# nagadomi/nunif

Measured on NVIDIA H100. Metric: waifu2x_input_megapixels_per_sec, higher is better.
Workload: dtype f16

## Files before the change

### nunif_b200/csrc/gemm_wgmma.cuh

```cuda
#pragma once
#include "common.cuh"
#include "ptx.cuh"
#include <cuda.h>

namespace nb200 {

enum : int { ACT_NONE = 0, ACT_LRELU01 = 1, ACT_GELU = 2, ACT_RELU = 3 };
enum : int { OUT_NHWC = 0, OUT_PIXSHUF2 = 1, OUT_SPLIT = 2 };

struct GemmParams {
    int B, Ho, Wo, TH, TW, tiles_x, tiles_y;
    int N;
    int taps, cpt;
    int8_t tap_dx[16], tap_dy[16], tap_dyi[16];
    int n_tiles;
    const float* bias;
    int act;
    int out_mode, cout;
    int has_res, res_cy, res_cx;
    int res_before_act;
    int k2;
};

struct GemmMaps {
    CUtensorMap a, b;
    CUtensorMap o[4];
    union {
        CUtensorMap r[4];
        CUtensorMap a2;
    };
};

__device__ __forceinline__ void mbar_init(uint64_t* bar, uint32_t count) {
    asm volatile("mbarrier.init.shared::cta.b64 [%0], %1;" ::"r"(smem_u32(bar)), "r"(count));
}
__device__ __forceinline__ void mbar_expect_tx(uint64_t* bar, uint32_t bytes) {
    asm volatile("mbarrier.arrive.expect_tx.shared::cta.b64 _, [%0], %1;" ::"r"(smem_u32(bar)), "r"(bytes) : "memory");
}
__device__ __forceinline__ void mbar_arrive(uint64_t* bar) {
    asm volatile("mbarrier.arrive.shared::cta.b64 _, [%0];" ::"r"(smem_u32(bar)) : "memory");
}
__device__ __forceinline__ void mbar_wait(uint64_t* bar, uint32_t parity) {
    const uint32_t addr = smem_u32(bar);
    uint32_t done = 0;
#pragma unroll 1
    for (uint32_t it = 0; it < (1u << 18) && !done; ++it)
        asm volatile(
            "{\n\t.reg .pred p;\n\t"
            "mbarrier.try_wait.parity.shared::cta.b64 p, [%1], %2, %3;\n\t"
            "selp.u32 %0, 1, 0, p;\n\t}"
            : "=r"(done) : "r"(addr), "r"(parity), "r"(20000u) : "memory");
    if (!done) __trap();
}
__device__ __forceinline__ void fence_barrier_init() {
    asm volatile("fence.mbarrier_init.release.cluster;" ::: "memory");
    asm volatile("fence.proxy.async.shared::cta;" ::: "memory");
}
__device__ __forceinline__ void tma_load_5d(const CUtensorMap* map, uint64_t* bar, void* dst, int c0, int c1, int c2, int c3, int c4) {
    asm volatile(
        "cp.async.bulk.tensor.5d.shared::cluster.global.tile.mbarrier::complete_tx::bytes [%0], [%1, {%3, %4, %5, %6, %7}], [%2];"
        ::"r"(smem_u32(dst)), "l"(map), "r"(smem_u32(bar)), "r"(c0), "r"(c1), "r"(c2), "r"(c3), "r"(c4) : "memory");
}
__device__ __forceinline__ void tma_load_2d(const CUtensorMap* map, uint64_t* bar, void* dst, int c0, int c1) {
    asm volatile(
        "cp.async.bulk.tensor.2d.shared::cluster.global.tile.mbarrier::complete_tx::bytes [%0], [%1, {%3, %4}], [%2];"
        ::"r"(smem_u32(dst)), "l"(map), "r"(smem_u32(bar)), "r"(c0), "r"(c1) : "memory");
}
__device__ __forceinline__ void tma_load_4d(const CUtensorMap* map, uint64_t* bar, void* dst, int c0, int c1, int c2, int c3) {
    asm volatile(
        "cp.async.bulk.tensor.4d.shared::cluster.global.tile.mbarrier::complete_tx::bytes [%0], [%1, {%3, %4, %5, %6}], [%2];"
        ::"r"(smem_u32(dst)), "l"(map), "r"(smem_u32(bar)), "r"(c0), "r"(c1), "r"(c2), "r"(c3) : "memory");
}
__device__ __forceinline__ void tma_store_4d(const CUtensorMap* map, const void* src, int c0, int c1, int c2, int c3) {
    asm volatile("cp.async.bulk.tensor.4d.global.shared::cta.tile.bulk_group [%0, {%2, %3, %4, %5}], [%1];"
                 ::"l"(map), "r"(smem_u32(src)), "r"(c0), "r"(c1), "r"(c2), "r"(c3) : "memory");
}
__device__ __forceinline__ void tma_store_2d(const CUtensorMap* map, const void* src, int c0, int c1) {
    asm volatile("cp.async.bulk.tensor.2d.global.shared::cta.tile.bulk_group [%0, {%2, %3}], [%1];"
                 ::"l"(map), "r"(smem_u32(src)), "r"(c0), "r"(c1) : "memory");
}
__device__ __forceinline__ void tma_store_commit() { asm volatile("cp.async.bulk.commit_group;" ::: "memory"); }
__device__ __forceinline__ void tma_store_wait_read() { asm volatile("cp.async.bulk.wait_group.read 0;" ::: "memory"); }
__device__ __forceinline__ void fence_async_smem() { asm volatile("fence.proxy.async.shared::cta;" ::: "memory"); }
__device__ __forceinline__ void consumer_bar_sync() { asm volatile("bar.sync 1, 256;" ::: "memory"); }
__device__ __forceinline__ void tma_prefetch_desc(const CUtensorMap* map) {
    asm volatile("prefetch.tensormap [%0];" ::"l"(map) : "memory");
}
__device__ __forceinline__ bool elect_one() {
    uint32_t pred;
    asm volatile(
        "{\n\t.reg .pred p;\n\t"
        "elect.sync _|p, 0xffffffff;\n\t"
        "selp.u32 %0, 1, 0, p;\n\t}"
        : "=r"(pred));
    return pred != 0;
}
__device__ __forceinline__ void wgmma_fence() { asm volatile("wgmma.fence.sync.aligned;" ::: "memory"); }
__device__ __forceinline__ void wgmma_commit() { asm volatile("wgmma.commit_group.sync.aligned;" ::: "memory"); }
template <int N>
__device__ __forceinline__ void wgmma_wait() { asm volatile("wgmma.wait_group.sync.aligned %0;" ::"n"(N) : "memory"); }
template <int K>
__device__ __forceinline__ void wgmma_fence_operands(float (&d)[K]) {
#pragma unroll
    for (int j = 0; j < K; ++j) asm volatile("" : "+f"(d[j])::"memory");
}

template <int SWIZZLE_BYTES>
__device__ __forceinline__ uint64_t make_kmajor_desc(uint32_t saddr) {
    constexpr uint64_t layout = SWIZZLE_BYTES == 128 ? 1 : (SWIZZLE_BYTES == 64 ? 2 : 3);
    constexpr uint64_t sbo = (8 * SWIZZLE_BYTES) >> 4;
    return (uint64_t)((saddr & 0x3FFFF) >> 4) | (1ull << 16) | (sbo << 32) | (layout << 62);
}

template <int N>
__device__ void wgmma_f16(float (&d)[N / 2], uint64_t a, uint64_t b, uint32_t acc);
template <> __device__ __forceinline__ void wgmma_f16<16>(float (&d)[8], uint64_t a, uint64_t b, uint32_t acc) {
    asm volatile("{\n\t.reg .pred p;\n\tsetp.ne.b32 p, %10, 0;\n\t"
                 "wgmma.mma_async.sync.aligned.m64n16k16.f32.f16.f16 {%0, %1, %2, %3, %4, %5, %6, %7}, %8, %9, p, 1, 1, 0, 0;\n\t}"
                 : "+f"(d[0]), "+f"(d[1]), "+f"(d[2]), "+f"(d[3]), "+f"(d[4]), "+f"(d[5]), "+f"(d[6]), "+f"(d[7])
                 : "l"(a), "l"(b), "r"(acc));
}
template <> __device__ __forceinline__ void wgmma_f16<32>(float (&d)[16], uint64_t a, uint64_t b, uint32_t acc) {
    asm volatile("{\n\t.reg .pred p;\n\tsetp.ne.b32 p, %18, 0;\n\t"
                 "wgmma.mma_async.sync.aligned.m64n32k16.f32.f16.f16 {%0, %1, %2, %3, %4, %5, %6, %7, %8, %9, %10, %11, %12, %13, %14, %15}, %16, %17, p, 1, 1, 0, 0;\n\t}"
                 : "+f"(d[0]), "+f"(d[1]), "+f"(d[2]), "+f"(d[3]), "+f"(d[4]), "+f"(d[5]), "+f"(d[6]), "+f"(d[7]), "+f"(d[8]), "+f"(d[9]), "+f"(d[10]), "+f"(d[11]), "+f"(d[12]), "+f"(d[13]), "+f"(d[14]), "+f"(d[15])
                 : "l"(a), "l"(b), "r"(acc));
}
template <> __device__ __forceinline__ void wgmma_f16<48>(float (&d)[24], uint64_t a, uint64_t b, uint32_t acc) {
    asm volatile("{\n\t.reg .pred p;\n\tsetp.ne.b32 p, %26, 0;\n\t"
                 "wgmma.mma_async.sync.aligned.m64n48k16.f32.f16.f16 {%0, %1, %2, %3, %4, %5, %6, %7, %8, %9, %10, %11, %12, %13, %14, %15, %16, %17, %18, %19, %20, %21, %22, %23}, %24, %25, p, 1, 1, 0, 0;\n\t}"
                 : "+f"(d[0]), "+f"(d[1]), "+f"(d[2]), "+f"(d[3]), "+f"(d[4]), "+f"(d[5]), "+f"(d[6]), "+f"(d[7]), "+f"(d[8]), "+f"(d[9]), "+f"(d[10]), "+f"(d[11]), "+f"(d[12]), "+f"(d[13]), "+f"(d[14]), "+f"(d[15]), "+f"(d[16]), "+f"(d[17]), "+f"(d[18]), "+f"(d[19]), "+f"(d[20]), "+f"(d[21]), "+f"(d[22]), "+f"(d[23])
                 : "l"(a), "l"(b), "r"(acc));
}
template <> __device__ __forceinline__ void wgmma_f16<64>(float (&d)[32], uint64_t a, uint64_t b, uint32_t acc) {
    asm volatile("{\n\t.reg .pred p;\n\tsetp.ne.b32 p, %34, 0;\n\t"
                 "wgmma.mma_async.sync.aligned.m64n64k16.f32.f16.f16 {%0, %1, %2, %3, %4, %5, %6, %7, %8, %9, %10, %11, %12, %13, %14, %15, %16, %17, %18, %19, %20, %21, %22, %23, %24, %25, %26, %27, %28, %29, %30, %31}, %32, %33, p, 1, 1, 0, 0;\n\t}"
                 : "+f"(d[0]), "+f"(d[1]), "+f"(d[2]), "+f"(d[3]), "+f"(d[4]), "+f"(d[5]), "+f"(d[6]), "+f"(d[7]), "+f"(d[8]), "+f"(d[9]), "+f"(d[10]), "+f"(d[11]), "+f"(d[12]), "+f"(d[13]), "+f"(d[14]), "+f"(d[15]), "+f"(d[16]), "+f"(d[17]), "+f"(d[18]), "+f"(d[19]), "+f"(d[20]), "+f"(d[21]), "+f"(d[22]), "+f"(d[23]), "+f"(d[24]), "+f"(d[25]), "+f"(d[26]), "+f"(d[27]), "+f"(d[28]), "+f"(d[29]), "+f"(d[30]), "+f"(d[31])
                 : "l"(a), "l"(b), "r"(acc));
}
template <> __device__ __forceinline__ void wgmma_f16<96>(float (&d)[48], uint64_t a, uint64_t b, uint32_t acc) {
    asm volatile("{\n\t.reg .pred p;\n\tsetp.ne.b32 p, %50, 0;\n\t"
                 "wgmma.mma_async.sync.aligned.m64n96k16.f32.f16.f16 {%0, %1, %2, %3, %4, %5, %6, %7, %8, %9, %10, %11, %12, %13, %14, %15, %16, %17, %18, %19, %20, %21, %22, %23, %24, %25, %26, %27, %28, %29, %30, %31, %32, %33, %34, %35, %36, %37, %38, %39, %40, %41, %42, %43, %44, %45, %46, %47}, %48, %49, p, 1, 1, 0, 0;\n\t}"
                 : "+f"(d[0]), "+f"(d[1]), "+f"(d[2]), "+f"(d[3]), "+f"(d[4]), "+f"(d[5]), "+f"(d[6]), "+f"(d[7]), "+f"(d[8]), "+f"(d[9]), "+f"(d[10]), "+f"(d[11]), "+f"(d[12]), "+f"(d[13]), "+f"(d[14]), "+f"(d[15]), "+f"(d[16]), "+f"(d[17]), "+f"(d[18]), "+f"(d[19]), "+f"(d[20]), "+f"(d[21]), "+f"(d[22]), "+f"(d[23]), "+f"(d[24]), "+f"(d[25]), "+f"(d[26]), "+f"(d[27]), "+f"(d[28]), "+f"(d[29]), "+f"(d[30]), "+f"(d[31]), "+f"(d[32]), "+f"(d[33]), "+f"(d[34]), "+f"(d[35]), "+f"(d[36]), "+f"(d[37]), "+f"(d[38]), "+f"(d[39]), "+f"(d[40]), "+f"(d[41]), "+f"(d[42]), "+f"(d[43]), "+f"(d[44]), "+f"(d[45]), "+f"(d[46]), "+f"(d[47])
                 : "l"(a), "l"(b), "r"(acc));
}
template <> __device__ __forceinline__ void wgmma_f16<128>(float (&d)[64], uint64_t a, uint64_t b, uint32_t acc) {
    asm volatile("{\n\t.reg .pred p;\n\tsetp.ne.b32 p, %66, 0;\n\t"
                 "wgmma.mma_async.sync.aligned.m64n128k16.f32.f16.f16 {%0, %1, %2, %3, %4, %5, %6, %7, %8, %9, %10, %11, %12, %13, %14, %15, %16, %17, %18, %19, %20, %21, %22, %23, %24, %25, %26, %27, %28, %29, %30, %31, %32, %33, %34, %35, %36, %37, %38, %39, %40, %41, %42, %43, %44, %45, %46, %47, %48, %49, %50, %51, %52, %53, %54, %55, %56, %57, %58, %59, %60, %61, %62, %63}, %64, %65, p, 1, 1, 0, 0;\n\t}"
                 : "+f"(d[0]), "+f"(d[1]), "+f"(d[2]), "+f"(d[3]), "+f"(d[4]), "+f"(d[5]), "+f"(d[6]), "+f"(d[7]), "+f"(d[8]), "+f"(d[9]), "+f"(d[10]), "+f"(d[11]), "+f"(d[12]), "+f"(d[13]), "+f"(d[14]), "+f"(d[15]), "+f"(d[16]), "+f"(d[17]), "+f"(d[18]), "+f"(d[19]), "+f"(d[20]), "+f"(d[21]), "+f"(d[22]), "+f"(d[23]), "+f"(d[24]), "+f"(d[25]), "+f"(d[26]), "+f"(d[27]), "+f"(d[28]), "+f"(d[29]), "+f"(d[30]), "+f"(d[31]), "+f"(d[32]), "+f"(d[33]), "+f"(d[34]), "+f"(d[35]), "+f"(d[36]), "+f"(d[37]), "+f"(d[38]), "+f"(d[39]), "+f"(d[40]), "+f"(d[41]), "+f"(d[42]), "+f"(d[43]), "+f"(d[44]), "+f"(d[45]), "+f"(d[46]), "+f"(d[47]), "+f"(d[48]), "+f"(d[49]), "+f"(d[50]), "+f"(d[51]), "+f"(d[52]), "+f"(d[53]), "+f"(d[54]), "+f"(d[55]), "+f"(d[56]), "+f"(d[57]), "+f"(d[58]), "+f"(d[59]), "+f"(d[60]), "+f"(d[61]), "+f"(d[62]), "+f"(d[63])
                 : "l"(a), "l"(b), "r"(acc));
}

__device__ __forceinline__ void wgmma_f16_rs96(float (&d)[48], const uint32_t (&a)[4], uint64_t b, uint32_t acc) {
    asm volatile("{\n\t.reg .pred p;\n\tsetp.ne.b32 p, %53, 0;\n\t"
                 "wgmma.mma_async.sync.aligned.m64n96k16.f32.f16.f16 {%0, %1, %2, %3, %4, %5, %6, %7, %8, %9, %10, %11, %12, %13, %14, %15, %16, %17, %18, %19, %20, %21, %22, %23, %24, %25, %26, %27, %28, %29, %30, %31, %32, %33, %34, %35, %36, %37, %38, %39, %40, %41, %42, %43, %44, %45, %46, %47}, {%48, %49, %50, %51}, %52, p, 1, 1, 0;\n\t}"
                 : "+f"(d[0]), "+f"(d[1]), "+f"(d[2]), "+f"(d[3]), "+f"(d[4]), "+f"(d[5]), "+f"(d[6]), "+f"(d[7]), "+f"(d[8]), "+f"(d[9]), "+f"(d[10]), "+f"(d[11]), "+f"(d[12]), "+f"(d[13]), "+f"(d[14]), "+f"(d[15]), "+f"(d[16]), "+f"(d[17]), "+f"(d[18]), "+f"(d[19]), "+f"(d[20]), "+f"(d[21]), "+f"(d[22]), "+f"(d[23]), "+f"(d[24]), "+f"(d[25]), "+f"(d[26]), "+f"(d[27]), "+f"(d[28]), "+f"(d[29]), "+f"(d[30]), "+f"(d[31]), "+f"(d[32]), "+f"(d[33]), "+f"(d[34]), "+f"(d[35]), "+f"(d[36]), "+f"(d[37]), "+f"(d[38]), "+f"(d[39]), "+f"(d[40]), "+f"(d[41]), "+f"(d[42]), "+f"(d[43]), "+f"(d[44]), "+f"(d[45]), "+f"(d[46]), "+f"(d[47])
                 : "r"(a[0]), "r"(a[1]), "r"(a[2]), "r"(a[3]), "l"(b), "r"(acc));
}

__device__ __forceinline__ float gelu_erf(float x) {
    const float a = fabsf(x);
    float q = fmaf(a, 4.88118734e-04f, -7.19881030e-03f);
    q = fmaf(q, a, 5.21468017e-02f);
    q = fmaf(q, a, 4.59595724e-01f);
    q = fmaf(q, a, 1.15100057e+00f);
    const float e = ex2(fmaf(-q, a, -1.0f));
    return fmaxf(x, 0.f) - a * e;
}

template <int K>
__device__ __forceinline__ void apply_act(float (&v)[K], int act) {
    switch (act) {
        case ACT_LRELU01:
#pragma unroll
            for (int j = 0; j < K; ++j) v[j] = v[j] > 0.f ? v[j] : 0.1f * v[j];
            break;
        case ACT_GELU:
#pragma unroll
            for (int j = 0; j < K; ++j) v[j] = gelu_erf(v[j]);
            break;
        case ACT_RELU:
#pragma unroll
            for (int j = 0; j < K; ++j) v[j] = fmaxf(v[j], 0.f);
            break;
        default: break;
    }
}

constexpr int GEMM_CONSUMER_THREADS = 256;
constexpr int GEMM_THREADS = GEMM_CONSUMER_THREADS + 32;

template <int BLOCK_N, int BK>
struct GemmCfg {
    static_assert(BLOCK_N % 16 == 0 && BLOCK_N <= 128, "BLOCK_N: 16..128 (the fp32 accumulators live in registers)");
    static constexpr int SWIZZLE = BK * 2;
    static constexpr int A_BYTES = 128 * BK * 2;
    static constexpr int B_BYTES = BLOCK_N * BK * 2;
    static constexpr int STAGE_BYTES = A_BYTES + ((B_BYTES + 1023) / 1024) * 1024;
    static constexpr int STAGES = (98304 / STAGE_BYTES) < 2 ? 2 : ((98304 / STAGE_BYTES) > 6 ? 6 : (98304 / STAGE_BYTES));
    static constexpr int CW = (BLOCK_N % 64 == 0) ? 64 : ((BLOCK_N % 32 == 0) ? 32 : 16);
    static constexpr int NCH = BLOCK_N / CW;
    static constexpr int CH_BYTES = 128 * CW * 2;
    static_assert(NCH * CH_BYTES <= STAGES * STAGE_BYTES, "epilogue staging must fit in the (drained) pipeline stages");
    static constexpr int SMEM_BYTES = STAGES * STAGE_BYTES + 1024  + 256 ;
};

template <int CW>
__device__ __forceinline__ uint32_t stage_off(int r, int j) {
    if (CW == 64) return (uint32_t)(r * 128 + ((j ^ (r & 7)) << 4));
    if (CW == 32) return (uint32_t)(r * 64 + ((j ^ ((r >> 1) & 3)) << 4));
    return (uint32_t)(r * 32 + ((j ^ ((r >> 2) & 1)) << 4));
}

template <int ROWS>
__device__ __forceinline__ uint32_t sw64_off(int r, int col) {
    return (uint32_t)((col >> 5) * (ROWS * 64)) + stage_off<32>(r, (col & 31) >> 3) + (uint32_t)((col & 7) * 2);
}

template <int BLOCK_N, int BK, bool A2 = false>
__global__ void __launch_bounds__(GEMM_THREADS, 2) gemm_conv_kernel(const __grid_constant__ GemmMaps maps,
                                                                    const __grid_constant__ GemmParams p) {
    using Cfg = GemmCfg<BLOCK_N, BK>;
    constexpr int STAGES = Cfg::STAGES;
    constexpr int CW = Cfg::CW;
    extern __shared__ uint8_t smem_dyn[];
    uint8_t* smem = reinterpret_cast<uint8_t*>((reinterpret_cast<uintptr_t>(smem_dyn) + 1023) & ~(uintptr_t)1023);
    uint64_t* full_bar = reinterpret_cast<uint64_t*>(smem + STAGES * Cfg::STAGE_BYTES);
    uint64_t* empty_bar = full_bar + STAGES;
    uint64_t* res_bar = empty_bar + STAGES;

    const int warp = threadIdx.x >> 5;
    const int n_tile = blockIdx.x % p.n_tiles;
    const int tile = blockIdx.x / p.n_tiles;
    const int tx_i = tile % p.tiles_x;
    const int ty_i = (tile / p.tiles_x) % p.tiles_y;
    const int b = tile / (p.tiles_x * p.tiles_y);
    const int x0 = tx_i * p.TW, y0 = ty_i * p.TH;
    const int n0 = n_tile * BLOCK_N;
    const int k_iters = p.taps * p.cpt + (A2 ? p.k2 : 0);

    if (threadIdx.x == GEMM_CONSUMER_THREADS) {
        tma_prefetch_desc(&maps.a);
        tma_prefetch_desc(&maps.b);
        tma_prefetch_desc(&maps.o[0]);
        for (int s = 0; s < STAGES; ++s) {
            mbar_init(&full_bar[s], 1);
            mbar_init(&empty_bar[s], 2);
        }
        mbar_init(res_bar, 1);
        fence_barrier_init();
    }
    __syncthreads();

    if (warp == GEMM_CONSUMER_THREADS / 32) {
        if (elect_one()) {
            asm volatile("griddepcontrol.wait;" ::: "memory");
            for (int it = 0; it < k_iters; ++it) {
                const int s = it % STAGES;
                const uint32_t ph = (it / STAGES) & 1;
                mbar_wait(&empty_bar[s], ph ^ 1);
                const int tap = it / p.cpt, ch = it - tap * p.cpt;
                uint8_t* sa = smem + s * Cfg::STAGE_BYTES;
                uint8_t* sb = sa + Cfg::A_BYTES;
                mbar_expect_tx(&full_bar[s], Cfg::A_BYTES + Cfg::B_BYTES);
                if (A2 && tap >= p.taps) {
                    const int q = n0 / p.cout;
                    tma_load_5d(&maps.a2, &full_bar[s], sa, (it - p.taps * p.cpt) * BK, q & 1, x0, q >> 1, b * p.Ho + y0);
                } else {
                    tma_load_5d(&maps.a, &full_bar[s], sa, ch * BK, x0 + p.tap_dx[tap], p.tap_dyi[tap], y0 + p.tap_dy[tap], b);
                }
                tma_load_2d(&maps.b, &full_bar[s], sb, it * BK, n0);
            }
        }
        return;
    }

    const int wg = threadIdx.x >> 7;
    const int t = threadIdx.x & 127;
    float acc[BLOCK_N / 2];
#pragma unroll
    for (int j = 0; j < BLOCK_N / 2; ++j) acc[j] = 0.f;
    for (int it = 0; it < k_iters; ++it) {
        const int s = it % STAGES;
        mbar_wait(&full_bar[s], (it / STAGES) & 1);
        const uint32_t sa = smem_u32(smem + s * Cfg::STAGE_BYTES) + wg * 64 * Cfg::SWIZZLE;
        const uint32_t sb = smem_u32(smem + s * Cfg::STAGE_BYTES) + Cfg::A_BYTES;
        wgmma_fence();
#pragma unroll
        for (int k = 0; k < BK / 16; ++k)
            wgmma_f16<BLOCK_N>(acc, make_kmajor_desc<Cfg::SWIZZLE>(sa + k * 32), make_kmajor_desc<Cfg::SWIZZLE>(sb + k * 32), 1u);
        wgmma_commit();
        wgmma_wait<1>();
        if (it > 0 && t == 0) mbar_arrive(&empty_bar[(it - 1) % STAGES]);
    }
    wgmma_wait<0>();
    wgmma_fence_operands(acc);
    if (threadIdx.x == 0) NB_PDL_TRIGGER();
    consumer_bar_sync();
    uint8_t* stg = smem;
    const bool leader = threadIdx.x == 0;
    if (p.has_res) {
        if (leader) {
            mbar_expect_tx(res_bar, Cfg::NCH * Cfg::CH_BYTES);
#pragma unroll 1
            for (int c = 0; c < Cfg::NCH; ++c) {
                const int n = n0 + c * CW;
                const int g = p.out_mode != OUT_NHWC ? n / p.cout : 0;
                const int co = p.out_mode != OUT_NHWC ? n - g * p.cout : n;
                tma_load_4d(&maps.r[g], res_bar, stg + c * Cfg::CH_BYTES, co, x0 + p.res_cx, y0 + p.res_cy, b);
            }
        }
        mbar_wait(res_bar, 0);
    }
    const int act = p.act;
    const bool has_res = p.has_res != 0, res_first = p.res_before_act != 0;
    const int row0 = wg * 64 + (t >> 5) * 16 + ((t & 31) >> 2);
    const int cq = 2 * (t & 3);
#pragma unroll
    for (int j = 0; j < BLOCK_N / 8; ++j) {
        const int col = 8 * j + cq;
        const int c = (8 * j) / CW;
        float2 bq = make_float2(0.f, 0.f);
        if (p.bias) bq = __ldg(reinterpret_cast<const float2*>(p.bias + n0 + col));
        float v[4] = {acc[4 * j] + bq.x, acc[4 * j + 1] + bq.y, acc[4 * j + 2] + bq.x, acc[4 * j + 3] + bq.y};
        __half2* s0 = reinterpret_cast<__half2*>(stg + c * Cfg::CH_BYTES + stage_off<CW>(row0, (8 * j % CW) / 8) + 2 * cq);
        __half2* s1 = reinterpret_cast<__half2*>(stg + c * Cfg::CH_BYTES + stage_off<CW>(row0 + 8, (8 * j % CW) / 8) + 2 * cq);
        if (has_res) {
            const float2 r0 = __half22float2(*s0), r1 = __half22float2(*s1);
            const float rv[4] = {r0.x, r0.y, r1.x, r1.y};
            if (res_first) {
#pragma unroll
                for (int q = 0; q < 4; ++q) v[q] += rv[q];
                apply_act(v, act);
            } else {
                apply_act(v, act);
#pragma unroll
                for (int q = 0; q < 4; ++q) v[q] += rv[q];
            }
        } else {
            apply_act(v, act);
        }
        *s0 = __floats2half2_rn(v[0], v[1]);
        *s1 = __floats2half2_rn(v[2], v[3]);
    }
    fence_async_smem();
    consumer_bar_sync();
    if (leader) {
#pragma unroll 1
        for (int c = 0; c < Cfg::NCH; ++c) {
            const int n = n0 + c * CW;
            const int g = p.out_mode != OUT_NHWC ? n / p.cout : 0;
            const int co = p.out_mode != OUT_NHWC ? n - g * p.cout : n;
            tma_store_4d(&maps.o[g], stg + c * Cfg::CH_BYTES, co, x0, y0, b);
        }
        tma_store_commit();
        tma_store_wait_read();
    }
}

}
```

### nunif_b200/csrc/swin_block.cu

```cuda
#include "gemm_wgmma.cuh"
#include "swin_kernels.h"
#include "tmap.h"
#include <algorithm>

namespace nb200 {

extern int g_tune[16];

constexpr int FM_ROWS = 128, FM_STAGES = 5, FM_THREADS = GEMM_CONSUMER_THREADS + 128;
constexpr int FM_PRODUCER_REGS = 40, FM_CONSUMER_REGS = 232;

template <int C>
struct FmCfg {
    static constexpr int KB = C / 32;
    static constexpr int NBUF = C == 96 ? 3 : 2;
    static constexpr int TILE = FM_ROWS * C * 2;
    static constexpr int STAGE = 128 * C;
    static constexpr int SMEM = NBUF * TILE + FM_STAGES * STAGE + (2 * FM_STAGES + NBUF * (KB + 2) + 1) * 8 + 1024;
    static_assert(SMEM <= 232448, "shared memory per CTA exceeds the opt-in limit");
};

struct FmMaps {
    CUtensorMap x, att, wp, w1, w2, y, wy;
};

template <int K>
__device__ __forceinline__ float (&half96(float (&acc)[K], int h))[48] { return *reinterpret_cast<float(*)[48]>(&acc[48 * h]); }

__device__ __forceinline__ void wgmma_wait_n(int n) {
    if (n == 0) wgmma_wait<0>();
    else wgmma_wait<1>();
}

template <int C, bool PROJ, int CS>
__global__ void __launch_bounds__(FM_THREADS, 1) swin_mlp_fused_kernel(const __grid_constant__ FmMaps maps, const float* __restrict__ bp,
                                                                     const float* __restrict__ b1, const float* __restrict__ b2,
                                                                     const float* __restrict__ by, int ntiles) {
    using Cfg = FmCfg<C>;
    static_assert(CS % 16 == 0 && 2 * C * CS <= Cfg::STAGE && CS * 256 <= Cfg::TILE, "Wy must fit a ring stage, y a tile");
    constexpr int KB = Cfg::KB, NP = (KB + 1) / 2, NH = 2 * C / 64, NHALF = C / 96, NBUF = Cfg::NBUF;
    constexpr int SPT = (PROJ ? NP : 0) + 2 * NH + (CS ? 1 : 0);
    static_assert(SPT > FM_STAGES, "the barrier protocol needs more stages per tile than the ring holds");
    constexpr int XAHEAD = PROJ ? NBUF - 1 : NBUF;
    extern __shared__ uint8_t smem_dyn[];
    uint8_t* smem = smem_dyn + ((1024u - (smem_u32(smem_dyn) & 1023u)) & 1023u);
    uint8_t* ring = smem + NBUF * Cfg::TILE;
    uint64_t* full = reinterpret_cast<uint64_t*>(ring + FM_STAGES * Cfg::STAGE);
    uint64_t* empty = full + FM_STAGES;
    uint64_t* abar = empty + FM_STAGES;
    uint64_t* xbar = abar + NBUF * KB;
    uint64_t* outw = xbar + NBUF;
    uint64_t* xfree = outw + NBUF;
    auto buf = [&](int b) { return smem + b * Cfg::TILE; };
    const int tid = threadIdx.x, warp = tid >> 5;
    const int nt = (ntiles - (int)blockIdx.x + (int)gridDim.x - 1) / (int)gridDim.x;
    if (tid == GEMM_CONSUMER_THREADS) {
        tma_prefetch_desc(&maps.x);
        tma_prefetch_desc(&maps.w1);
        tma_prefetch_desc(&maps.w2);
        if (CS) {
            tma_prefetch_desc(&maps.wy);
            tma_prefetch_desc(&maps.y);
        }
        if (PROJ) {
            tma_prefetch_desc(&maps.att);
            tma_prefetch_desc(&maps.wp);
        }
        for (int s = 0; s < FM_STAGES; ++s) {
            mbar_init(&full[s], 1);
            mbar_init(&empty[s], 2);
        }
        for (int b = 0; b < NBUF; ++b) {
            for (int kb = 0; kb < KB; ++kb) mbar_init(&abar[b * KB + kb], 1);
            mbar_init(&xbar[b], 1);
            mbar_init(&outw[b], 2);
        }
        mbar_init(xfree, 2);
        fence_barrier_init();
    }
    __syncthreads();

    if (warp >= GEMM_CONSUMER_THREADS / 32) {
        asm volatile("setmaxnreg.dec.sync.aligned.u32 %0;" ::"n"(FM_PRODUCER_REGS));
        if (warp == GEMM_CONSUMER_THREADS / 32 && elect_one()) {
            int it = 0;
            auto push = [&](const CUtensorMap* m, int k0, int n0, int rows, int nbox) {
                const int s = it % FM_STAGES;
                mbar_wait(&empty[s], ((it / FM_STAGES) & 1) ^ 1);
                mbar_expect_tx(&full[s], nbox * rows * 64);
                for (int b = 0; b < nbox; ++b) tma_load_2d(m, &full[s], ring + s * Cfg::STAGE + b * rows * 64, k0 + 32 * b, n0);
                ++it;
            };
            for (int j = 0; j < nt; ++j) {
                if (PROJ)
                    for (int p = 0; p < NP; ++p) push(&maps.wp, 64 * p, 0, C, min(2, KB - 2 * p));
                push(&maps.w1, 0, 0, 64, KB);
                for (int hc = 0; hc < NH; ++hc) {
                    if (hc + 1 < NH) push(&maps.w1, 0, (hc + 1) * 64, 64, KB);
                    push(&maps.w2, hc * 64, 0, C, 2);
                }
                if (CS) push(&maps.wy, 0, 0, CS, KB);
            }
        } else if (warp == GEMM_CONSUMER_THREADS / 32 + 1 && elect_one()) {
            auto row = [&](int j) { return ((int)blockIdx.x + j * (int)gridDim.x) * FM_ROWS; };
            auto load_att = [&](int j) {
                const int b = j % NBUF;
                for (int kb = 0; kb < KB; ++kb) {
                    mbar_expect_tx(&abar[b * KB + kb], FM_ROWS * 64);
                    tma_load_2d(&maps.att, &abar[b * KB + kb], buf(b) + kb * (FM_ROWS * 64), kb * 32, row(j));
                }
            };
            auto load_x = [&](int j) {
                uint8_t* dst = buf((j + PROJ) % NBUF);
                mbar_expect_tx(&xbar[j % NBUF], Cfg::TILE);
                for (int kb = 0; kb < KB; ++kb) tma_load_2d(&maps.x, &xbar[j % NBUF], dst + kb * (FM_ROWS * 64), kb * 32, row(j));
            };
            asm volatile("griddepcontrol.wait;" ::: "memory");
            if (PROJ) load_att(0);
            for (int j = 0; j < XAHEAD && j < nt; ++j) load_x(j);
            for (int j = 0; j < nt; ++j) {
                if (PROJ) {
                    mbar_wait(xfree, j & 1);
                    if (j + 1 < nt) load_att(j + 1);
                }
                const int b = j % NBUF;
                mbar_wait(&outw[b], (j / NBUF) & 1);
                if constexpr (CS > 0)
                    for (int c = 0; c < CS / 16; ++c) tma_store_2d(&maps.y, buf(b) + c * (FM_ROWS * 32), 16 * c, row(j));
                else
                    for (int kb = 0; kb < KB; ++kb) tma_store_2d(&maps.x, buf(b) + kb * (FM_ROWS * 64), kb * 32, row(j));
                tma_store_commit();
                tma_store_wait_read();
                if (j + XAHEAD < nt) load_x(j + XAHEAD);
            }
        }
        return;
    }

    asm volatile("setmaxnreg.inc.sync.aligned.u32 %0;" ::"n"(FM_CONSUMER_REGS));
    const int wg = tid >> 7, t = tid & 127;
    const int row0 = wg * 64 + (t >> 5) * 16 + ((t & 31) >> 2);
    const int cq = 2 * (t & 3);
#pragma unroll 1
    for (int it0 = 0; (int)blockIdx.x + it0 / SPT * (int)gridDim.x < ntiles; it0 += SPT) {
        const int j = it0 / SPT;
        int it = it0;
        const int b = j % NBUF;
        const uint32_t par = (j / NBUF) & 1;
        uint8_t* sx1 = buf(b);
        const uint8_t* sxin = buf((j + PROJ) % NBUF);
        const uint32_t x1_base = smem_u32(sx1) + wg * 64 * 64;
        int pending = 0;
        auto take = [&]() -> uint32_t {
            const int s = it % FM_STAGES;
            mbar_wait(&full[s], (it / FM_STAGES) & 1);
            return smem_u32(ring + s * Cfg::STAGE);
        };
        auto commit = [&]() {
            wgmma_commit();
            ++it;
            ++pending;
        };
        auto retire = [&](int n) {
            wgmma_wait_n(n);
#pragma unroll
            for (int k = 0; k < FM_STAGES; ++k)
                if (k < pending - n && t == 0) mbar_arrive(&empty[(it - pending + k) % FM_STAGES]);
            pending = min(pending, n);
        };

        if (PROJ) {
            float acc[C / 2];
#pragma unroll
            for (int i = 0; i < C / 2; ++i) acc[i] = 0.f;
            wgmma_fence_operands(acc);
#pragma unroll
            for (int p = 0; p < NP; ++p) {
                const uint32_t bb = take();
#pragma unroll
                for (int kb = 2 * p; kb < 2 * p + 2 && kb < KB; ++kb) mbar_wait(&abar[b * KB + kb], par);
                wgmma_fence();
#pragma unroll
                for (int kb = 2 * p; kb < 2 * p + 2 && kb < KB; ++kb) {
                    const uint32_t a = x1_base + kb * (FM_ROWS * 64), w = bb + (kb - 2 * p) * (C * 64);
#pragma unroll
                    for (int s = 0; s < 2; ++s)
#pragma unroll
                        for (int h = 0; h < NHALF; ++h)
                            wgmma_f16<96>(half96(acc, h), make_kmajor_desc<64>(a + 32 * s), make_kmajor_desc<64>(w + h * 96 * 64 + 32 * s), 1u);
                }
                commit();
                retire(1);
            }
            retire(0);
            wgmma_fence_operands(acc);
            mbar_wait(&xbar[b], par);
#pragma unroll
            for (int q = 0; q < C / 8; ++q) {
                const int col = 8 * q + cq;
                const float2 bq = __ldg(reinterpret_cast<const float2*>(bp + col));
#pragma unroll
                for (int i = 0; i < 2; ++i) {
                    const uint32_t off = sw64_off<FM_ROWS>(row0 + 8 * i, col);
                    const float2 xv = __half22float2(*reinterpret_cast<const __half2*>(sxin + off));
                    *reinterpret_cast<__half2*>(sx1 + off) =
                        __floats2half2_rn(xv.x + (acc[4 * q + 2 * i] + bq.x), xv.y + (acc[4 * q + 2 * i + 1] + bq.y));
                }
            }
            fence_async_smem();
            asm volatile("bar.sync %0, 128;" ::"r"(2 + wg) : "memory");
            if (t == 0) mbar_arrive(xfree);
        } else {
            mbar_wait(&xbar[b], par);
        }

        float oacc[C / 2];
#pragma unroll
        for (int i = 0; i < C / 2; ++i) oacc[i] = 0.f;
        wgmma_fence_operands(oacc);
        float hacc[2][32];
        uint32_t af[4][4];
        auto fc1 = [&](float (&h)[32]) {
#pragma unroll
            for (int i = 0; i < 32; ++i) h[i] = 0.f;
            wgmma_fence_operands(h);
            const uint32_t bb = take();
            wgmma_fence();
#pragma unroll
            for (int kb = 0; kb < KB; ++kb) {
                const uint32_t a = x1_base + kb * (FM_ROWS * 64), w = bb + kb * (64 * 64);
                wgmma_f16<64>(h, make_kmajor_desc<64>(a), make_kmajor_desc<64>(w), 1u);
                wgmma_f16<64>(h, make_kmajor_desc<64>(a + 32), make_kmajor_desc<64>(w + 32), 1u);
            }
            commit();
        };
        fc1(hacc[0]);
#pragma unroll
        for (int hc = 0; hc < NH; ++hc) {
            const int hb = hc & 1;
            if (hc + 1 < NH) fc1(hacc[hb ^ 1]);
            retire(hc + 1 < NH ? 1 : 0);
            wgmma_fence_operands(hacc[hb]);
#pragma unroll
            for (int kk = 0; kk < 4; ++kk)
#pragma unroll
                for (int q = 0; q < 4; ++q) {
                    const int c8 = 2 * kk + (q >> 1), i = q & 1;
                    const float2 bq = __ldg(reinterpret_cast<const float2*>(b1 + 64 * hc + 8 * c8 + cq));
                    af[kk][q] = pack_half2(gelu_erf(hacc[hb][4 * c8 + 2 * i] + bq.x), gelu_erf(hacc[hb][4 * c8 + 2 * i + 1] + bq.y));
                }
            const uint32_t bb = take();
            wgmma_fence();
#pragma unroll
            for (int kb = 0; kb < 2; ++kb)
#pragma unroll
                for (int s = 0; s < 2; ++s)
#pragma unroll
                    for (int h = 0; h < NHALF; ++h)
                        wgmma_f16_rs96(half96(oacc, h), af[2 * kb + s], make_kmajor_desc<64>(bb + kb * (C * 64) + h * 96 * 64 + 32 * s), 1u);
            commit();
        }
        retire(0);
        wgmma_fence_operands(oacc);
#pragma unroll
        for (int q = 0; q < C / 8; ++q) {
            const int col = 8 * q + cq;
            const float2 bq = __ldg(reinterpret_cast<const float2*>(b2 + col));
#pragma unroll
            for (int i = 0; i < 2; ++i) {
                __half2* p = reinterpret_cast<__half2*>(sx1 + sw64_off<FM_ROWS>(row0 + 8 * i, col));
                const float2 xv = __half22float2(*p);
                *p = __floats2half2_rn(xv.x + (oacc[4 * q + 2 * i] + bq.x), xv.y + (oacc[4 * q + 2 * i + 1] + bq.y));
            }
        }
        fence_async_smem();
        if constexpr (CS > 0) {
            asm volatile("bar.sync %0, 128;" ::"r"(2 + wg) : "memory");
            float yacc[CS / 2];
#pragma unroll
            for (int i = 0; i < CS / 2; ++i) yacc[i] = 0.f;
            wgmma_fence_operands(yacc);
            const uint32_t bb = take();
            wgmma_fence();
#pragma unroll
            for (int kb = 0; kb < KB; ++kb) {
                const uint32_t a = x1_base + kb * (FM_ROWS * 64), w = bb + kb * (CS * 64);
                wgmma_f16<CS>(yacc, make_kmajor_desc<64>(a), make_kmajor_desc<64>(w), 1u);
                wgmma_f16<CS>(yacc, make_kmajor_desc<64>(a + 32), make_kmajor_desc<64>(w + 32), 1u);
            }
            commit();
            retire(0);
            wgmma_fence_operands(yacc);
            consumer_bar_sync();
#pragma unroll
            for (int q = 0; q < CS / 8; ++q) {
                const int col = 8 * q + cq;
                const float2 bq = __ldg(reinterpret_cast<const float2*>(by + col));
#pragma unroll
                for (int i = 0; i < 2; ++i) {
                    __half2* p = reinterpret_cast<__half2*>(sx1 + (col >> 4) * (FM_ROWS * 32) + stage_off<16>(row0 + 8 * i, (col & 15) >> 3) +
                                                            (col & 7) * 2);
                    *p = __floats2half2_rn(yacc[4 * q + 2 * i] + bq.x, yacc[4 * q + 2 * i + 1] + bq.y);
                }
            }
            fence_async_smem();
        }
        asm volatile("bar.sync %0, 128;" ::"r"(2 + wg) : "memory");
        if (t == 0) mbar_arrive(&outw[b]);
    }
}

static int map2d(CUtensorMap* m, const void* base, int cols, long long rows, int box_rows) {
    const cuuint64_t dims[2] = {(cuuint64_t)cols, (cuuint64_t)rows};
    const cuuint64_t strides[1] = {(cuuint64_t)cols * 2};
    const cuuint32_t box[2] = {32, (cuuint32_t)box_rows};
    return encode(m, base, 2, dims, strides, box, 64);
}

template <int C, bool PROJ, int CS = 0>
static int launch_mlp(cudaStream_t st, int ntiles, const FmMaps& maps, const float* bp, const float* b1, const float* b2,
                      const float* by = nullptr) {
    if (ensure_dyn_smem((const void*)swin_mlp_fused_kernel<C, PROJ, CS>, FmCfg<C>::SMEM)) return 1;
    cudaLaunchConfig_t cfg = {};
    int grid = std::min(ntiles, device_sm_count());
    if (g_tune[10] > 0) grid = std::min(grid, g_tune[10]);
    cfg.gridDim = dim3((unsigned)grid); cfg.blockDim = dim3(FM_THREADS); cfg.dynamicSmemBytes = FmCfg<C>::SMEM;
    cfg.stream = st;
    cudaLaunchAttribute at[1];
    at[0].id = cudaLaunchAttributeProgrammaticStreamSerialization;
    at[0].val.programmaticStreamSerializationAllowed = 1;
    cfg.attrs = at; cfg.numAttrs = 1;
    NB_CUDA(cudaLaunchKernelEx(&cfg, swin_mlp_fused_kernel<C, PROJ, CS>, maps, bp, b1, b2, by, ntiles));
    NB_LAUNCHED();
    return 0;
}

int swin_mlp_fused(cudaStream_t st, __half* x, const __half* att, long long T, int C, const __half* wp, const float* bp,
                   const __half* w1, const float* b1, const __half* w2, const float* b2, __half* y, int cs, const __half* wy,
                   const float* by) {
    NB_CHECK(x && w1 && b1 && w2 && b2 && (!att || (wp && bp)) && (!y || (att && wy && by)), "null pointer");
    NB_CHECK(C == 96 || C == 192, "C must be 96 or 192");
    NB_CHECK(!y || (C == 192 && cs == 48) || (C == 96 && cs == 16), "y: cs must be 48 at C = 192 and 16 at C = 96");
    NB_CHECK(T > 0 && T < (1LL << 31), "token count out of range");
    FmMaps maps;
    memset(&maps, 0, sizeof(maps));
    if (map2d(&maps.x, x, C, T, FM_ROWS)) return 1;
    if (att && (map2d(&maps.att, att, C, T, FM_ROWS) || map2d(&maps.wp, wp, C, C, C))) return 1;
    if (map2d(&maps.w1, w1, C, 2 * C, 64) || map2d(&maps.w2, w2, 2 * C, C, C)) return 1;
    if (y) {
        if (map2d(&maps.wy, wy, C, cs, cs)) return 1;
        const cuuint64_t dims[2] = {(cuuint64_t)cs, (cuuint64_t)T};
        const cuuint64_t strides[1] = {(cuuint64_t)cs * 2};
        const cuuint32_t box[2] = {16, FM_ROWS};
        if (encode(&maps.y, y, 2, dims, strides, box, 32)) return 1;
    }
    const double Td = (double)T;
    ProfScope ps(st, PC_FUSED_MLP, Td * C * 2 * (C * ((att ? 1 : 0) + 4) + (y ? cs : 0)), Td * C * 2 * (att ? 2 : 1),
                 Td * (y ? cs : C) * 2);
    const int ntiles = (int)((T + FM_ROWS - 1) / FM_ROWS);
    if (rec_on()) rec_launch("swin_mlp", {{"T", T}, {"C", C}, {"proj", att ? 1 : 0}, {"cs", y ? cs : 0}});
    if (y) return C == 96 ? launch_mlp<96, true, 16>(st, ntiles, maps, bp, b1, b2, by) : launch_mlp<192, true, 48>(st, ntiles, maps, bp, b1, b2, by);
    if (C == 96) return att ? launch_mlp<96, true>(st, ntiles, maps, bp, b1, b2) : launch_mlp<96, false>(st, ntiles, maps, bp, b1, b2);
    return att ? launch_mlp<192, true>(st, ntiles, maps, bp, b1, b2) : launch_mlp<192, false>(st, ntiles, maps, bp, b1, b2);
}

}

using namespace nb200;

extern "C" int nb200_swin_mlp_fused_f16(void* x, const void* att, long long T, int C, const void* wp, const float* bp,
                                        const void* w1, const float* b1, const void* w2, const float* b2, void* stream) {
    return swin_mlp_fused((cudaStream_t)stream, (__half*)x, (const __half*)att, T, C, (const __half*)wp, bp, (const __half*)w1, b1,
                          (const __half*)w2, b2, nullptr, 0, nullptr, nullptr);
}

extern "C" int nb200_swin_mlp_fused_y_f16(void* x, const void* att, long long T, int C, const void* wp, const float* bp,
                                          const void* w1, const float* b1, const void* w2, const float* b2, void* y, int cs,
                                          const void* wy, const float* by, void* stream) {
    NB_CHECK(y, "null pointer");
    return swin_mlp_fused((cudaStream_t)stream, (__half*)x, (const __half*)att, T, C, (const __half*)wp, bp, (const __half*)w1, b1,
                          (const __half*)w2, b2, (__half*)y, cs, (const __half*)wy, by);
}
```

Before: 81.19.

## Multicast MLP weight tiles across 2-CTA clusters and stage biases in shared memory

Launches the fused Swin MLP kernel as two-CTA clusters. Each CTA issues half of the weight TMA boxes with cluster multicast, and consumers release ring stages on both CTAs' empty barriers, which halves L2 weight traffic per pair. Biases are copied into shared memory once per CTA instead of being read with __ldg in the epilogues. The cost is cross-CTA coupling: the two CTAs must advance through the weight ring in lockstep, a drain wait is added before exit, and the grid is sized from cluster occupancy, so some SMs may be left idle.

```diff
diff --git a/nunif_b200/csrc/gemm_wgmma.cuh b/nunif_b200/csrc/gemm_wgmma.cuh
--- a/nunif_b200/csrc/gemm_wgmma.cuh
+++ b/nunif_b200/csrc/gemm_wgmma.cuh
@@ -52,6 +52,20 @@
             : "=r"(done) : "r"(addr), "r"(parity), "r"(20000u) : "memory");
     if (!done) __trap();
 }
+__device__ __forceinline__ uint32_t cluster_ctarank() {
+    uint32_t r;
+    asm volatile("mov.u32 %0, %%cluster_ctarank;" : "=r"(r));
+    return r;
+}
+__device__ __forceinline__ void mbar_arrive_cluster(uint64_t* bar, uint32_t cta) {
+    asm volatile(
+        "{\n\t.reg .b32 ra;\n\t"
+        "mapa.shared::cluster.u32 ra, %0, %1;\n\t"
+        "mbarrier.arrive.shared::cluster.b64 _, [ra];\n\t}"
+        ::"r"(smem_u32(bar)), "r"(cta) : "memory");
+}
+__device__ __forceinline__ void cluster_arrive() { asm volatile("barrier.cluster.arrive.release;" ::: "memory"); }
+__device__ __forceinline__ void cluster_wait() { asm volatile("barrier.cluster.wait.acquire;" ::: "memory"); }
 __device__ __forceinline__ void fence_barrier_init() {
     asm volatile("fence.mbarrier_init.release.cluster;" ::: "memory");
     asm volatile("fence.proxy.async.shared::cta;" ::: "memory");
@@ -65,6 +79,12 @@
     asm volatile(
         "cp.async.bulk.tensor.2d.shared::cluster.global.tile.mbarrier::complete_tx::bytes [%0], [%1, {%3, %4}], [%2];"
         ::"r"(smem_u32(dst)), "l"(map), "r"(smem_u32(bar)), "r"(c0), "r"(c1) : "memory");
+}
+__device__ __forceinline__ void tma_load_2d_multicast(const CUtensorMap* map, uint64_t* bar, void* dst, int c0, int c1,
+                                                      uint16_t cta_mask) {
+    asm volatile(
+        "cp.async.bulk.tensor.2d.shared::cluster.global.tile.mbarrier::complete_tx::bytes.multicast::cluster [%0], [%1, {%3, %4}], [%2], %5;"
+        ::"r"(smem_u32(dst)), "l"(map), "r"(smem_u32(bar)), "r"(c0), "r"(c1), "h"(cta_mask) : "memory");
 }
 __device__ __forceinline__ void tma_load_4d(const CUtensorMap* map, uint64_t* bar, void* dst, int c0, int c1, int c2, int c3) {
     asm volatile(
diff --git a/nunif_b200/csrc/swin_block.cu b/nunif_b200/csrc/swin_block.cu
--- a/nunif_b200/csrc/swin_block.cu
+++ b/nunif_b200/csrc/swin_block.cu
@@ -2,12 +2,14 @@
 #include "swin_kernels.h"
 #include "tmap.h"
 #include <algorithm>
+#include <atomic>
 
 namespace nb200 {
 
 extern int g_tune[16];
 
 constexpr int FM_ROWS = 128, FM_STAGES = 5, FM_THREADS = GEMM_CONSUMER_THREADS + 128;
+constexpr int FM_CLUSTER = 2;
 constexpr int FM_PRODUCER_REGS = 40, FM_CONSUMER_REGS = 232;
 
 template <int C>
@@ -16,7 +18,8 @@
     static constexpr int NBUF = C == 96 ? 3 : 2;
     static constexpr int TILE = FM_ROWS * C * 2;
     static constexpr int STAGE = 128 * C;
-    static constexpr int SMEM = NBUF * TILE + FM_STAGES * STAGE + (2 * FM_STAGES + NBUF * (KB + 2) + 1) * 8 + 1024;
+    static constexpr int BIAS = 4 * C + 64;
+    static constexpr int SMEM = NBUF * TILE + FM_STAGES * STAGE + (2 * FM_STAGES + NBUF * (KB + 2) + 1) * 8 + BIAS * 4 + 1024;
     static_assert(SMEM <= 232448, "shared memory per CTA exceeds the opt-in limit");
 };
 
@@ -38,6 +41,8 @@
                                                                      const float* __restrict__ by, int ntiles) {
     using Cfg = FmCfg<C>;
     static_assert(CS % 16 == 0 && 2 * C * CS <= Cfg::STAGE && CS * 256 <= Cfg::TILE, "Wy must fit a ring stage, y a tile");
+    static_assert(PROJ || CS == 0, "y needs att");
+    static_assert(CS <= 64, "by must fit its shared-memory slot");
     constexpr int KB = Cfg::KB, NP = (KB + 1) / 2, NH = 2 * C / 64, NHALF = C / 96, NBUF = Cfg::NBUF;
     constexpr int SPT = (PROJ ? NP : 0) + 2 * NH + (CS ? 1 : 0);
     static_assert(SPT > FM_STAGES, "the barrier protocol needs more stages per tile than the ring holds");
@@ -51,9 +56,13 @@
     uint64_t* xbar = abar + NBUF * KB;
     uint64_t* outw = xbar + NBUF;
     uint64_t* xfree = outw + NBUF;
+    float* sbp = reinterpret_cast<float*>(xfree + 1);
+    float* sb1 = sbp + C;
+    float* sb2 = sb1 + 2 * C;
+    float* sby = sb2 + C;
     auto buf = [&](int b) { return smem + b * Cfg::TILE; };
     const int tid = threadIdx.x, warp = tid >> 5;
-    const int nt = (ntiles - (int)blockIdx.x + (int)gridDim.x - 1) / (int)gridDim.x;
+    const int nt = (ntiles - (int)(blockIdx.x & ~1u) + (int)gridDim.x - 1) / (int)gridDim.x;
     if (tid == GEMM_CONSUMER_THREADS) {
         tma_prefetch_desc(&maps.x);
         tma_prefetch_desc(&maps.w1);
@@ -68,7 +77,7 @@
         }
         for (int s = 0; s < FM_STAGES; ++s) {
             mbar_init(&full[s], 1);
-            mbar_init(&empty[s], 2);
+            mbar_init(&empty[s], 2 * FM_CLUSTER);
         }
         for (int b = 0; b < NBUF; ++b) {
             for (int kb = 0; kb < KB; ++kb) mbar_init(&abar[b * KB + kb], 1);
@@ -78,17 +87,28 @@
         mbar_init(xfree, 2);
         fence_barrier_init();
     }
-    __syncthreads();
+    for (int i = tid; i < 2 * C; i += FM_THREADS) {
+        sb1[i] = b1[i];
+        if (i < C) {
+            sb2[i] = b2[i];
+            if (PROJ) sbp[i] = bp[i];
+        }
+        if (CS > 0 && i < CS) sby[i] = by[i];
+    }
+    cluster_arrive();
+    cluster_wait();
 
     if (warp >= GEMM_CONSUMER_THREADS / 32) {
         asm volatile("setmaxnreg.dec.sync.aligned.u32 %0;" ::"n"(FM_PRODUCER_REGS));
         if (warp == GEMM_CONSUMER_THREADS / 32 && elect_one()) {
             int it = 0;
+            const int rank = (int)cluster_ctarank();
             auto push = [&](const CUtensorMap* m, int k0, int n0, int rows, int nbox) {
                 const int s = it % FM_STAGES;
                 mbar_wait(&empty[s], ((it / FM_STAGES) & 1) ^ 1);
                 mbar_expect_tx(&full[s], nbox * rows * 64);
-                for (int b = 0; b < nbox; ++b) tma_load_2d(m, &full[s], ring + s * Cfg::STAGE + b * rows * 64, k0 + 32 * b, n0);
+                for (int b = rank; b < nbox; b += FM_CLUSTER)
+                    tma_load_2d_multicast(m, &full[s], ring + s * Cfg::STAGE + b * rows * 64, k0 + 32 * b, n0, (1u << FM_CLUSTER) - 1);
                 ++it;
             };
             for (int j = 0; j < nt; ++j) {
@@ -101,6 +121,7 @@
                 }
                 if (CS) push(&maps.wy, 0, 0, CS, KB);
             }
+            for (int q = max(it - FM_STAGES, 0); q < it; ++q) mbar_wait(&empty[q % FM_STAGES], (q / FM_STAGES) & 1);
         } else if (warp == GEMM_CONSUMER_THREADS / 32 + 1 && elect_one()) {
             auto row = [&](int j) { return ((int)blockIdx.x + j * (int)gridDim.x) * FM_ROWS; };
             auto load_att = [&](int j) {
@@ -142,7 +163,7 @@
     const int row0 = wg * 64 + (t >> 5) * 16 + ((t & 31) >> 2);
     const int cq = 2 * (t & 3);
 #pragma unroll 1
-    for (int it0 = 0; (int)blockIdx.x + it0 / SPT * (int)gridDim.x < ntiles; it0 += SPT) {
+    for (int it0 = 0; (int)(blockIdx.x & ~1u) + it0 / SPT * (int)gridDim.x < ntiles; it0 += SPT) {
         const int j = it0 / SPT;
         int it = it0;
         const int b = j % NBUF;
@@ -165,7 +186,10 @@
             wgmma_wait_n(n);
 #pragma unroll
             for (int k = 0; k < FM_STAGES; ++k)
-                if (k < pending - n && t == 0) mbar_arrive(&empty[(it - pending + k) % FM_STAGES]);
+                if (k < pending - n && t == 0) {
+                    mbar_arrive_cluster(&empty[(it - pending + k) % FM_STAGES], 0);
+                    mbar_arrive_cluster(&empty[(it - pending + k) % FM_STAGES], 1);
+                }
             pending = min(pending, n);
         };
 
@@ -198,7 +222,7 @@
 #pragma unroll
             for (int q = 0; q < C / 8; ++q) {
                 const int col = 8 * q + cq;
-                const float2 bq = __ldg(reinterpret_cast<const float2*>(bp + col));
+                const float2 bq = *reinterpret_cast<const float2*>(sbp + col);
 #pragma unroll
                 for (int i = 0; i < 2; ++i) {
                     const uint32_t off = sw64_off<FM_ROWS>(row0 + 8 * i, col);
@@ -246,7 +270,7 @@
 #pragma unroll
                 for (int q = 0; q < 4; ++q) {
                     const int c8 = 2 * kk + (q >> 1), i = q & 1;
-                    const float2 bq = __ldg(reinterpret_cast<const float2*>(b1 + 64 * hc + 8 * c8 + cq));
+                    const float2 bq = *reinterpret_cast<const float2*>(sb1 + 64 * hc + 8 * c8 + cq);
                     af[kk][q] = pack_half2(gelu_erf(hacc[hb][4 * c8 + 2 * i] + bq.x), gelu_erf(hacc[hb][4 * c8 + 2 * i + 1] + bq.y));
                 }
             const uint32_t bb = take();
@@ -265,7 +289,7 @@
 #pragma unroll
         for (int q = 0; q < C / 8; ++q) {
             const int col = 8 * q + cq;
-            const float2 bq = __ldg(reinterpret_cast<const float2*>(b2 + col));
+            const float2 bq = *reinterpret_cast<const float2*>(sb2 + col);
 #pragma unroll
             for (int i = 0; i < 2; ++i) {
                 __half2* p = reinterpret_cast<__half2*>(sx1 + sw64_off<FM_ROWS>(row0 + 8 * i, col));
@@ -295,7 +319,7 @@
 #pragma unroll
             for (int q = 0; q < CS / 8; ++q) {
                 const int col = 8 * q + cq;
-                const float2 bq = __ldg(reinterpret_cast<const float2*>(by + col));
+                const float2 bq = *reinterpret_cast<const float2*>(sby + col);
 #pragma unroll
                 for (int i = 0; i < 2; ++i) {
                     __half2* p = reinterpret_cast<__half2*>(sx1 + (col >> 4) * (FM_ROWS * 32) + stage_off<16>(row0 + 8 * i, (col & 15) >> 3) +
@@ -320,16 +344,31 @@
 template <int C, bool PROJ, int CS = 0>
 static int launch_mlp(cudaStream_t st, int ntiles, const FmMaps& maps, const float* bp, const float* b1, const float* b2,
                       const float* by = nullptr) {
-    if (ensure_dyn_smem((const void*)swin_mlp_fused_kernel<C, PROJ, CS>, FmCfg<C>::SMEM)) return 1;
+    const void* fn = (const void*)swin_mlp_fused_kernel<C, PROJ, CS>;
+    if (ensure_dyn_smem(fn, FmCfg<C>::SMEM)) return 1;
     cudaLaunchConfig_t cfg = {};
-    int grid = std::min(ntiles, device_sm_count());
-    if (g_tune[10] > 0) grid = std::min(grid, g_tune[10]);
-    cfg.gridDim = dim3((unsigned)grid); cfg.blockDim = dim3(FM_THREADS); cfg.dynamicSmemBytes = FmCfg<C>::SMEM;
+    cfg.blockDim = dim3(FM_THREADS); cfg.dynamicSmemBytes = FmCfg<C>::SMEM;
     cfg.stream = st;
-    cudaLaunchAttribute at[1];
+    cudaLaunchAttribute at[2];
     at[0].id = cudaLaunchAttributeProgrammaticStreamSerialization;
     at[0].val.programmaticStreamSerializationAllowed = 1;
-    cfg.attrs = at; cfg.numAttrs = 1;
+    at[1].id = cudaLaunchAttributeClusterDimension;
+    at[1].val.clusterDim.x = FM_CLUSTER; at[1].val.clusterDim.y = 1; at[1].val.clusterDim.z = 1;
+    cfg.attrs = at; cfg.numAttrs = 2;
+    static std::atomic<int> max_clusters[64];
+    int dev = 0;
+    NB_CUDA(cudaGetDevice(&dev));
+    std::atomic<int>& mc = max_clusters[dev >= 0 && dev < 64 ? dev : 0];
+    int ncl = mc.load(std::memory_order_relaxed);
+    if (ncl <= 0) {
+        cfg.gridDim = dim3((unsigned)(FM_CLUSTER * device_sm_count()));
+        NB_CUDA(cudaOccupancyMaxActiveClusters(&ncl, fn, &cfg));
+        NB_CHECK(ncl > 0, "swin_mlp_fused_kernel: no cluster of two CTAs fits on this device");
+        mc.store(ncl, std::memory_order_relaxed);
+    }
+    ncl = std::min(ncl, (ntiles + FM_CLUSTER - 1) / FM_CLUSTER);
+    if (g_tune[10] > 0) ncl = std::min(ncl, std::max(g_tune[10] / FM_CLUSTER, 1));
+    cfg.gridDim = dim3((unsigned)(FM_CLUSTER * ncl));
     NB_CUDA(cudaLaunchKernelEx(&cfg, swin_mlp_fused_kernel<C, PROJ, CS>, maps, bp, b1, b2, by, ntiles));
     NB_LAUNCHED();
     return 0;
@@ -341,7 +380,7 @@
     NB_CHECK(x && w1 && b1 && w2 && b2 && (!att || (wp && bp)) && (!y || (att && wy && by)), "null pointer");
     NB_CHECK(C == 96 || C == 192, "C must be 96 or 192");
     NB_CHECK(!y || (C == 192 && cs == 48) || (C == 96 && cs == 16), "y: cs must be 48 at C = 192 and 16 at C = 96");
-    NB_CHECK(T > 0 && T < (1LL << 31), "token count out of range");
+    NB_CHECK(T > 0 && T < (1LL << 31) - FM_ROWS, "token count out of range");
     FmMaps maps;
     memset(&maps, 0, sizeof(maps));
     if (map2d(&maps.x, x, C, T, FM_ROWS)) return 1;
```

Result: faster. 82.13 (median of 6 runs) (+1.2%).
